# philip-bl/dctn

Measured on AMD Instinct MI355X. Metric: EPS-contraction windows/sec (fwd+bwd), higher is better.
Workload: dtype bf16; 1 GPU; cfg2 EPS[(3,4)]+linear bf16 B1024/GPU; parallelism=dp1

## Files before the change

### dctn_amd/csrc/eps_mfma.hip

```cpp
#include "common.h"

#include <cstdlib>
#include <type_traits>

typedef __attribute__((ext_vector_type(8))) __bf16 bf16x8;
typedef __attribute__((ext_vector_type(16))) float f32x16;
typedef __attribute__((ext_vector_type(8))) float f32x8;
typedef __attribute__((ext_vector_type(2))) int int2v;
typedef __attribute__((ext_vector_type(4))) int int4v;
typedef __attribute__((ext_vector_type(2))) float f32x2;

namespace {

constexpr int ilog2(int v) { return v <= 1 ? 0 : 1 + ilog2(v >> 1); }

template <typename S> __device__ __forceinline__ float to_f32(S v) { return (float)v; }

__device__ __forceinline__ float half_sum(float v) {
  const int iv = __float_as_int(v);
  const int2v r = __builtin_amdgcn_permlane32_swap(iv, iv, false, false);
  return __int_as_float(r[0]) + __int_as_float(r[1]);
}

__device__ __forceinline__ void swap_halves(float& a, float& b) {
// ... 47 lines not shown

struct FastDiv {
  unsigned M, s1, s2;
};
__device__ __forceinline__ unsigned fdiv(unsigned n, const FastDiv& d) {
  const unsigned t = __umulhi(d.M, n);
  return (t + ((n - t) >> d.s1)) >> d.s2;
}

#define MFMA_MAXN 16
struct MfmaP {
  int C, B, K, O, Ho, Wo;
  int P;
  int npg;
  int spc, nchunks;
  unsigned foffb[MFMA_MAXN];
  unsigned rowoffb[MFMA_MAXN];
  unsigned s1b, s2b, s3b, s4b;
  unsigned x_bytes;
  unsigned o_bytes, o_s1b;
  FastDiv div_wo;
  int rowvec_ok;
  int vec_ok;
  int Cout;
  unsigned hw_rowb, hw_bytes;
  int ncb;
  int opts;
#ifdef DCTN_STAMPS
  unsigned long long* stamps;
#endif
};

#ifdef DCTN_STAMPS
#define DCTN_STAMP(P, SLOT)                                                                      \
  do {                                                                                           \
    __builtin_amdgcn_sched_barrier(0);                                                           \
    unsigned long long t_;                                                                       \
    asm volatile("s_memrealtime %0\n\ts_waitcnt lgkmcnt(0)" : "=s"(t_)::"memory");               \
    if ((P).stamps && threadIdx.x == 0) (P).stamps[(long long)blockIdx.x * 8 + (SLOT)] = t_;     \
    __builtin_amdgcn_sched_barrier(0);                                                           \
  } while (0)
static unsigned long long* g_stamps = nullptr;
void dctn_stamps_set(unsigned long long* p) { g_stamps = p; }
__device__ unsigned long long* g_dev_stamps = nullptr;
void dctn_reduce_stamps_set(unsigned long long* p) { (void)hipMemcpyToSymbol(HIP_SYMBOL(g_dev_stamps), &p, sizeof(p)); }
#define DCTN_STAMP_T(P, SLOT, TID)                                                              \
  do {                                                                                           \
    __builtin_amdgcn_sched_barrier(0);                                                           \
    unsigned long long t_;                                                                       \
    asm volatile("s_memrealtime %0\n\ts_waitcnt lgkmcnt(0)" : "=s"(t_)::"memory");               \
    if ((P).stamps && threadIdx.x == (TID)) (P).stamps[(long long)blockIdx.x * 8 + (SLOT)] = t_;  \
    __builtin_amdgcn_sched_barrier(0);                                                           \
  } while (0)
#define DCTN_STAMP_G(SLOT)                                                                       \
  do {                                                                                           \
    __builtin_amdgcn_sched_barrier(0);                                                           \
    unsigned long long t_;                                                                       \
    asm volatile("s_memrealtime %0\n\ts_waitcnt lgkmcnt(0)" : "=s"(t_)::"memory");               \
    if (g_dev_stamps && threadIdx.x == 0) g_dev_stamps[(long long)blockIdx.x * 8 + (SLOT)] = t_;  \
    __builtin_amdgcn_sched_barrier(0);                                                           \
  } while (0)
#else
#define DCTN_STAMP(P, SLOT) do { } while (0)
#define DCTN_STAMP_T(P, SLOT, TID) do { } while (0)
#define DCTN_STAMP_G(SLOT) do { } while (0)
#endif

typedef __attribute__((ext_vector_type(4))) unsigned u32x4;
typedef __attribute__((ext_vector_type(2))) unsigned u32x2;
typedef __attribute__((ext_vector_type(2))) __bf16 bf16x2;

__device__ __forceinline__ __amdgpu_buffer_rsrc_t make_rsrc(const void* ptr, unsigned bytes) {
  return __builtin_amdgcn_make_buffer_rsrc(const_cast<void*>(ptr), 0, (int)bytes, 0x00020000);
}

template <typename S, int N, bool VEC, int ROWS>
struct RawWindow {
  u32x4 row[ROWS > 0 ? ROWS : 1];
  unsigned v[(ROWS == 0 && VEC) ? N * (int)(sizeof(S) / 2) : 1];
  unsigned e[(ROWS == 0 && !VEC) ? 2 * N : 1];
};

template <typename S, int N, bool VEC, int ROWS>
__device__ __forceinline__ void issue_window(__amdgpu_buffer_rsrc_t rs, unsigned voff, unsigned soff,
                                             const MfmaP& p, RawWindow<S, N, VEC, ROWS>& raw) {
  if constexpr (ROWS > 0) {
#pragma unroll
    for (int rw = 0; rw < ROWS; ++rw)
      raw.row[rw] = __builtin_amdgcn_raw_buffer_load_b128(rs, voff, soff + p.rowoffb[rw], 0);
  } else if constexpr (VEC) {
#pragma unroll
    for (int n = 0; n < N; ++n) {
      if constexpr (sizeof(S) == 2) {
        raw.v[n] = __builtin_amdgcn_raw_buffer_load_b32(rs, voff, soff + p.foffb[n], 0);
      } else {
        const u32x2 t = __builtin_amdgcn_raw_buffer_load_b64(rs, voff, soff + p.foffb[n], 0);
        raw.v[2 * n] = t.x;
        raw.v[2 * n + 1] = t.y;
      }
    }
  } else {
#pragma unroll
    for (int n = 0; n < N; ++n)
#pragma unroll
      for (int q = 0; q < 2; ++q) {
        if constexpr (sizeof(S) == 2)
          raw.e[2 * n + q] = (unsigned)(unsigned short)__builtin_amdgcn_raw_buffer_load_b16(
              rs, voff, soff + p.foffb[n] + q * p.s4b, 0);
        else
          raw.e[2 * n + q] = __builtin_amdgcn_raw_buffer_load_b32(rs, voff, soff + p.foffb[n] + q * p.s4b, 0);
      }
  }
}

template <typename S, int N, bool VEC, int ROWS>
__device__ __forceinline__ void unpack_window(const RawWindow<S, N, VEC, ROWS>& raw, float (&xv)[N][2]) {
  if constexpr (ROWS > 0) {
    constexpr int KK = N / ROWS;
// ... 672 lines not shown
    const int nks = (F + 31) / 32;
    const int c = lane & 15, kg = lane >> 4;
    const __amdgpu_buffer_rsrc_t rs_hw = make_rsrc(hw, p.hw_bytes);
    u32x4 wf[HEADT_MAXKS];
#pragma unroll
    for (int i = 0; i < HEADT_MAXKS; ++i) {
      const int ks = wv + HEADT_WAVES * i, k = 32 * ks + 8 * kg;
      const unsigned vo2 = (ks < nks && c < p.Cout && k + 7 < F) ? (unsigned)c * p.hw_rowb + (unsigned)k * 2u : p.hw_bytes;
      wf[i] = __builtin_amdgcn_raw_buffer_load_b128(rs_hw, vo2, 0, 0);
    }
    __syncthreads();
    f32x4v hd = {0.f, 0.f, 0.f, 0.f};
    const short* brd = ftile + (c < HEADT_GS ? c : HEADT_GS - 1) * LP + 8 * kg;
#pragma unroll
    for (int i = 0; i < HEADT_MAXKS; ++i) {
      const int ks = wv + HEADT_WAVES * i;
      if (ks < nks) {
        const bf16x8 fb = *reinterpret_cast<const bf16x8*>(brd + 32 * ks);
        hd = __builtin_amdgcn_mfma_f32_16x16x32_bf16(__builtin_bit_cast(bf16x8, wf[i]), fb, hd, 0, 0, 0);
      }
    }
    if (c < HEADT_GS) {
#pragma unroll
      for (int v = 0; v < 4; ++v) hsum[wv][c][4 * kg + v] = hd[v];
    }
    if constexpr (BLK4) {
      static_assert(HEADT_GS == 4, "a group is one block of the blocked4 layout");
      const unsigned sob = (unsigned)(g0 >> 2) * (unsigned)F * 8u;
      for (int f = 2 * tid; f < F; f += 2 * 64 * HEADT_WAVES) {
        unsigned r[HEADT_GS];
#pragma unroll
        for (int i = 0; i < HEADT_GS; ++i) r[i] = i < ng ? *reinterpret_cast<const unsigned*>(ftile + i * LP + f) : 0u;
        const u32x4 q = u32x4{__builtin_amdgcn_perm(r[1], r[0], 0x05040100u), __builtin_amdgcn_perm(r[3], r[2], 0x05040100u),
                              __builtin_amdgcn_perm(r[1], r[0], 0x07060302u), __builtin_amdgcn_perm(r[3], r[2], 0x07060302u)};
        __builtin_amdgcn_raw_buffer_store_b128(q, rs_o, (unsigned)f * 8u, sob, 0);
      }
    }
    __syncthreads();
    if (tid < HEADT_GS * 16) {
      const int sl = tid >> 4, cc = tid & 15;
      if (sl < ng && cc < p.Cout) {
        float t = (float)bias[cc];
#pragma unroll
        for (int w = 0; w < HEADT_WAVES; ++w) t += hsum[w][sl][cc];
        logits[(long long)(g0 + sl) * p.Cout + cc] = (bf16_t)t;
      }
    }
  }
}

constexpr int BWD_WAVES = 8;
constexpr size_t dcore_dyn_lds_bytes(int mt) { return (size_t)BWD_WAVES * (1 + mt) * 64 * 32 * sizeof(short); }

template <typename S, int N0, int N1, int OP, bool XVEC, bool OVEC, int ROWS, int HEADC>
__global__ __launch_bounds__(64 * BWD_WAVES) void eps_bwd_dcore_q2reg_k(const S* __restrict__ x,
                                                             const S* __restrict__ dY,
                                                             const S* __restrict__ hw,
                                                             const S* __restrict__ feat,
                                                             float* __restrict__ partial,
                                                             float* __restrict__ dwpart, MfmaP p) {
  constexpr int N = N0 + N1, A = 1 << N0, BN = 1 << N1, KS = A / 16, MT = BN * OP / 32;
  constexpr int AT = A >= 32 ? A / 32 : 1;
  constexpr int LOGO = ilog2(OP);
  constexpr bool LDST = A == 32 && MT <= 2;
  __shared__ float red[BWD_WAVES][32 * 32];
  extern __shared__ __attribute__((aligned(16))) unsigned char dsm[];
  const int tid = threadIdx.x, lane = tid & 63, r = lane & 31, h = lane >> 5, wv = tid >> 6;
  DCTN_STAMP(p, 0);
  short* tiles = reinterpret_cast<short*>(dsm) + wv * ((1 + MT) * 64 * LROW);
  const TrLane trl = tr_lane(lane);

  bf16x8 ident[2];
#pragma unroll
  for (int sp = 0; sp < 2; ++sp)
#pragma unroll
    for (int j = 0; j < 8; ++j) ident[sp][j] = (bf16_t)((16 * sp + 8 * h + j == r) ? 1.f : 0.f);

  f32x16 acc[MT][AT];
#pragma unroll
  for (int t = 0; t < MT; ++t)
#pragma unroll
    for (int a = 0; a < AT; ++a)
#pragma unroll
      for (int v = 0; v < 16; ++v) acc[t][a][v] = 0.f;

  const WaveJob job = wave_job(p, BWD_WAVES, (int)sizeof(S), HEADC > 0);
  const __amdgpu_buffer_rsrc_t rs_x = make_rsrc(x, p.x_bytes);
  const __amdgpu_buffer_rsrc_t rs_dy = make_rsrc(HEADC > 0 ? feat : dY, p.o_bytes);
  constexpr bool HEADMM = HEADC > 0 && HEADC <= 16 && LDST && OVEC && XVEC && sizeof(S) == 2 && OP == 4;
  float hwf[HEADC > 0 && !HEADMM ? HEADC : 1][OP];
  float dwacc[HEADC > 0 && !HEADMM ? HEADC : 1][OP];
#pragma unroll
  for (int c = 0; c < (HEADC > 0 && !HEADMM ? HEADC : 1); ++c)
#pragma unroll
    for (int o = 0; o < OP; ++o) dwacc[c][o] = 0.f;
  constexpr int DLW = HEADC > 0 ? HEADC / 2 : 1;
  const unsigned* dl32 = reinterpret_cast<const unsigned*>(dY);
  unsigned dlraw[DLW];
  RawRow<S, OP> rr[HEADC > 0 && !HEADMM ? HEADC : 1];
  constexpr bool LATE = HEADC > 0 && LDST && !HEADMM;
  auto issue_head_weight = [&]() {
    if constexpr (HEADC > 0 && !HEADMM) {
      const __amdgpu_buffer_rsrc_t rs_hw = make_rsrc(hw, p.hw_bytes);
      const unsigned voff_hw = job.valid ? (unsigned)job.pos * (unsigned)(OP * 2) : p.hw_bytes;
#pragma unroll
      for (int c = 0; c < HEADC; ++c)
        issue_row<S, OP, true>(rs_hw, c < p.Cout ? voff_hw : p.hw_bytes, (unsigned)c * p.hw_rowb, OP, rr[c]);
    }
  };
  auto ldst_step = [&](const float (&xv)[N][2], auto&& make_dy) {
    if constexpr (LDST) {
      bf16x8 X[KS], Y[KS];
      build_p0<N0>(xv, X, Y);
      float p1[BN];
      p1[0] = xv[N - 1][0];
      p1[1] = xv[N - 1][1];
#pragma unroll
      for (int u = 1; u < N1; ++u)
#pragma unroll
        for (int bb = (1 << u) - 1; bb >= 0; --bb) {
          const f32x2 pr = bmul2(p1[bb], f32x2{xv[N - 1 - u][0], xv[N - 1 - u][1]});
// ... 330 lines not shown
#pragma unroll
        for (int o = 0; o < OP; ++o) {
          float v = 0.f;
#pragma unroll
          for (int c = 0; c < HEADC; ++c) v = (c == c0 + cc) ? dwacc[c][o] : v;
          red1[wv * SLOT + (cc * 64 + lane) * OP + o] = v;
        }
      __syncthreads();
      for (int e = tid; e < CPR * 64 * OP; e += 64 * BWD_WAVES) {
        float sum = 0.f;
#pragma unroll
        for (int k = 0; k < BWD_WAVES; ++k) sum += red1[k * SLOT + e];
        const int cc = e / (64 * OP), rem = e - cc * (64 * OP);
        const int c = c0 + cc, f = pg * 64 * OP + rem;
        if (cb < p.ncb && c < p.Cout && f < F) dwpart[((long long)cb * p.Cout + c) * F + f] = sum;
      }
    }
  }
  DCTN_STAMP(p, 5);
}

template <typename S>
__global__ __launch_bounds__(256) void eps_bwd_dcore_reduce_k(const float* __restrict__ partial,
                                                              S* __restrict__ dCore, int nblk, int A,
                                                              int BN, int O, int OP, int ACOLS) {
  __shared__ float red[8][32];
  const int tid = threadIdx.x, c = tid & 31, k8 = tid >> 5;
  const long long stride = (long long)BN * OP * ACOLS;
  const long long e = (long long)blockIdx.x * 32 + c;
  float acc[8];
#pragma unroll
  for (int i = 0; i < 8; ++i) acc[i] = 0.f;
  int k = k8;
  for (; k + 56 < nblk; k += 64) {
#pragma unroll
    for (int i = 0; i < 8; ++i) acc[i] += partial[(k + 8 * i) * stride + e];
  }
  for (; k < nblk; k += 8) acc[0] += partial[k * stride + e];
  red[k8][c] = ((acc[0] + acc[1]) + (acc[2] + acc[3])) + ((acc[4] + acc[5]) + (acc[6] + acc[7]));
  __syncthreads();
  if (k8 == 0) {
    float t = 0.f;
#pragma unroll
    for (int i = 0; i < 8; ++i) t += red[i][c];
    const int m = (int)(e / ACOLS), a = (int)(e % ACOLS);
    const int b = m / OP, o = m % OP;
    if (a < A && o < O) dCore[((long long)a * BN + b) * O + o] = (S)t;
  }
}

constexpr int DWG_WAVES = 16;
constexpr int DWG_FW = 32;
constexpr int DWG_BFW = 16;
template <int FW, bool BLK4>
__device__ __forceinline__ void head_dw_gemm_role(const bf16_t* __restrict__ feat, const bf16_t* __restrict__ dL,
                                                  bf16_t* __restrict__ dW, int B, int Cout, long long F, int blk,
                                                  float* __restrict__ lds) {
  typedef __attribute__((ext_vector_type(4))) float f32x4v;
  constexpr int FL = FW / 16;
  static_assert(!BLK4 || FL == 1 || FL == 2, "blocked4 pieces of 8 or 16 bytes");
  const int tid = threadIdx.x, lane = tid & 63, wv = tid >> 6, n = lane & 15, kg = lane >> 4;
  const long long fb = BLK4 ? (long long)(B + 3) / 4 * 4 * F * 2 : (long long)B * F * 2;
  const unsigned f_bytes = (unsigned)fb, dl_bytes = (unsigned)B * (unsigned)Cout * 2u;
  const __amdgpu_buffer_rsrc_t rs_f = make_rsrc(feat, f_bytes), rs_dl = make_rsrc(dL, dl_bytes);
  const long long fcol = (long long)blk * FW + FL * n;
  const bool fok = fcol + FL - 1 < F;
  const int spw = (((B + DWG_WAVES - 1) / DWG_WAVES) + 31) / 32 * 32;
  const int b0 = wv * spw, b1 = b0 + spw < B ? b0 + spw : B;
  f32x4v acc[FL];
#pragma unroll
  for (int j = 0; j < FL; ++j) acc[j] = f32x4v{0.f, 0.f, 0.f, 0.f};
  constexpr int FD = FL >= 2 ? FL / 2 : 1;
  constexpr int NF = BLK4 ? 2 : 8, ND = BLK4 ? 2 * FL : FD;
  unsigned fr[NF][ND], frn[NF][ND];
  unsigned a16[8], a16n[8];
  auto issue = [&](int kb, unsigned (&f)[NF][ND], unsigned (&a)[8]) {
    if constexpr (BLK4) {
#pragma unroll
      for (int h = 0; h < 2; ++h) {
        const int b = kb + 8 * kg + 4 * h;
        const unsigned vo = (b < b1 && fok) ? (unsigned)(((long long)(b >> 2) * F + fcol) * 8) : f_bytes;
        if constexpr (FL == 1) {
          const u32x2 q = __builtin_amdgcn_raw_buffer_load_b64(rs_f, vo, 0, 0);
          f[h][0] = q.x;
          f[h][ND - 1] = q.y;
        } else {
          const u32x4 q = __builtin_amdgcn_raw_buffer_load_b128(rs_f, vo, 0, 0);
#pragma unroll
          for (int d = 0; d < 4; ++d) f[h][d] = q[d];
        }
      }
    }
#pragma unroll
    for (int j = 0; j < 8; ++j) {
      const int b = kb + 8 * kg + j;
      const bool in = b < b1;
      if constexpr (!BLK4) {
        const unsigned vo = (in && fok) ? (unsigned)((long long)b * F * 2 + fcol * 2) : f_bytes;
        if constexpr (FL == 1) {
          f[j][0] = (unsigned)(unsigned short)__builtin_amdgcn_raw_buffer_load_b16(rs_f, vo, 0, 0);
        } else if constexpr (FL == 2) {
          f[j][0] = __builtin_amdgcn_raw_buffer_load_b32(rs_f, vo, 0, 0);
        } else {
          const u32x2 q = __builtin_amdgcn_raw_buffer_load_b64(rs_f, vo, 0, 0);
          f[j][0] = q.x;
          f[j][FD - 1] = q.y;
        }
      }
      a[j] = (unsigned)(unsigned short)__builtin_amdgcn_raw_buffer_load_b16(
          rs_dl, (in && n < Cout) ? (unsigned)b * (unsigned)Cout * 2u + 2u * n : dl_bytes, 0, 0);
    }
  };
  DCTN_STAMP_G(0);
  if (b0 < b1) issue(b0, fr, a16);
  for (int kb = b0; kb < b1; kb += 32) {
    if (kb + 32 < b1) issue(kb + 32, frn, a16n);
    __builtin_amdgcn_sched_barrier(0);
    int4v at;
#pragma unroll
    for (int d = 0; d < 4; ++d) at[d] = (int)(a16[2 * d] | (a16[2 * d + 1] << 16));
#pragma unroll
    for (int j = 0; j < FL; ++j) {
      int4v bf;
      if constexpr (BLK4) {
#pragma unroll
        for (int d = 0; d < 4; ++d) bf[d] = (int)fr[d >> 1][2 * j + (d & 1)];
      } else {
        const unsigned sel = (j & 1) ? 0x07060302u : 0x05040100u;
#pragma unroll
        for (int d = 0; d < 4; ++d)
          bf[d] = FL == 1 ? (int)(fr[2 * d][0] | (fr[2 * d + 1][0] << 16))
                          : (int)__builtin_amdgcn_perm(fr[2 * d + 1][j >> 1], fr[2 * d][j >> 1], sel);
      }
      acc[j] = __builtin_amdgcn_mfma_f32_16x16x32_bf16(__builtin_bit_cast(bf16x8, at), __builtin_bit_cast(bf16x8, bf), acc[j], 0, 0, 0);
    }
#pragma unroll
    for (int j = 0; j < NF; ++j)
#pragma unroll
      for (int e = 0; e < ND; ++e) fr[j][e] = frn[j][e];
#pragma unroll
    for (int j = 0; j < 8; ++j) a16[j] = a16n[j];
  }
#pragma unroll
  for (int j = 0; j < FL; ++j)
#pragma unroll
    for (int i = 0; i < 4; ++i) lds[(wv * (4 * FL) + j * 4 + i) * 64 + lane] = acc[j][i];
  DCTN_STAMP_G(1);
  __syncthreads();
  DCTN_STAMP_G(2);
  if (tid < 4 * FL * 64) {
    const int slot = tid >> 6, j = slot >> 2, i = slot & 3;
    float t = 0.f;
#pragma unroll
    for (int w = 0; w < DWG_WAVES; ++w) t += lds[(w * (4 * FL) + slot) * 64 + lane];
    const int c = 4 * kg + i;
    const long long f = (long long)blk * FW + FL * n + j;
    if (c < Cout && f < F) dW[(long long)c * F + f] = (bf16_t)t;
  }
  DCTN_STAMP_G(4);
}

__global__ __launch_bounds__(1024) void eps_head_reduce_k(const float* __restrict__ partial,
                                                          bf16_t* __restrict__ dCore, int nblk, int A, int BN,
                                                          int O, int OP, int ACOLS, int n_core,
                                                          const float* __restrict__ dwpart,
                                                          bf16_t* __restrict__ dW, int ncb, long long nW, int n_dw,
                                                          const bf16_t* __restrict__ dL,
                                                          bf16_t* __restrict__ dBias, int B, int Cout,
                                                          const bf16_t* __restrict__ feat, int gemm) {
  __shared__ float red[32][33];
  const int tid = threadIdx.x;
  const int bid = gemm == 2 && (int)blockIdx.x < n_core + n_dw
                      ? ((int)blockIdx.x < n_dw ? n_core + (int)blockIdx.x : (int)blockIdx.x - n_dw)
                      : (int)blockIdx.x;
  if (bid < n_core) {
    DCTN_STAMP_G(0);
    const int c = tid & 31, k32 = tid >> 5;
    const long long stride = (long long)BN * OP * ACOLS;
    const long long e = (long long)bid * 32 + c;
    float acc = 0.f;
    for (int k0 = 0; k0 < nblk; k0 += 256) {
      float v[8];
#pragma unroll
      for (int i = 0; i < 8; ++i) {
        const int k = k0 + k32 + 32 * i;
        const float ld = partial[(k < nblk ? k : nblk - 1) * stride + e];
        v[i] = k < nblk ? ld : 0.f;
      }
      acc += ((v[0] + v[1]) + (v[2] + v[3])) + ((v[4] + v[5]) + (v[6] + v[7]));
    }
    red[k32][c] = acc;
    __syncthreads();
    if (k32 == 0) {
      float t = 0.f;
#pragma unroll
      for (int i = 0; i < 32; ++i) t += red[i][c];
      const int m = (int)(e / ACOLS), a = (int)(e % ACOLS);
      const int b = m / OP, o = m % OP;
      if (a < A && o < O) dCore[((long long)a * BN + b) * O + o] = (bf16_t)t;
    }
    DCTN_STAMP_G(4);
    return;
  }
  if (bid < n_core + n_dw) {
    if (!dW) return;
    if (gemm) {
      extern __shared__ __attribute__((aligned(16))) float gemm_lds[];
      if (gemm == 2) head_dw_gemm_role<DWG_BFW, true>(feat, dL, dW, B, Cout, nW / Cout, bid - n_core, gemm_lds);
      else head_dw_gemm_role<DWG_FW, false>(feat, dL, dW, B, Cout, nW / Cout, bid - n_core, gemm_lds);
      return;
    }
    const long long e = (long long)(bid - n_core) * 256 + (tid >> 2);
// ... 133 lines not shown
  if (chunks < 1) chunks = 1;
  if (chunks > m.B) chunks = m.B;
  m.spc = (int)((m.B + chunks - 1) / chunks);
  m.nchunks = (m.B + m.spc - 1) / m.spc;
  const long long waves = (long long)m.nchunks * m.npg;
  long long blocks = (waves + wpb - 1) / wpb;
  if (blocks >= 8) blocks = (blocks + 7) / 8 * 8;
  return (int)blocks;
}

template <typename S>
bool row_vec_ok(const MfmaP& m, int OP, const void* ptr) {
  return m.O == OP && ((uintptr_t)ptr % 4) == 0 && (OP * sizeof(S)) % 4 == 0;
}

template <typename S, int N0, int N1, int OP>
int fwd_launch_t(const void* x, const void* core, void* out, double* stats, const MfmaP& m_in, hipStream_t st) {
  MfmaP m = m_in;
  const int blocks = plan_waves(m, 4, (long long)FWD_BLOCKS_PER_CU * dctn_dev().cus * 4);
  const bool ovec = out == nullptr || row_vec_ok<S>(m, OP, out);
  const dim3 g((unsigned)blocks), b(256);
  constexpr int NN = N0 + N1;
  constexpr int RW = NN == 9 ? 3 : 4;
  if (m.rowvec_ok && m.vec_ok && ovec && sizeof(S) == 2)
    hipLaunchKernelGGL((eps_fwd_q2reg_k<S, N0, N1, OP, true, true, RW>), g, b, 0, st, (const S*)x,
                       (const S*)core, (S*)out, stats, m);
  else if (m.vec_ok && ovec)
    hipLaunchKernelGGL((eps_fwd_q2reg_k<S, N0, N1, OP, true, true, 0>), g, b, 0, st, (const S*)x,
                       (const S*)core, (S*)out, stats, m);
  else if (m.vec_ok)
    hipLaunchKernelGGL((eps_fwd_q2reg_k<S, N0, N1, OP, true, false, 0>), g, b, 0, st, (const S*)x,
                       (const S*)core, (S*)out, stats, m);
  else
    hipLaunchKernelGGL((eps_fwd_q2reg_k<S, N0, N1, OP, false, false, 0>), g, b, 0, st, (const S*)x,
                       (const S*)core, (S*)out, stats, m);
  DCTN_CHECK_LAUNCH();
  dctn_set_last_kernel("eps_fwd_mfma_q2reg");
  return DCTN_OK;
}

template <typename S, int N0, int N1, int OP>
int bwd_launch_t(const void* x, const void* dY, void* dCore, void* ws, const MfmaP& m_in,
                 hipStream_t st) {
  constexpr int A = 1 << N0, BN = 1 << N1, AT = A >= 32 ? A / 32 : 1;
  constexpr size_t DYN = dcore_dyn_lds<N0, N1, OP>();
  MfmaP m = m_in;
  const int grid = plan_waves(m, BWD_WAVES, (long long)dctn_dev().cus * BWD_WAVES);
  const bool ovec = row_vec_ok<S>(m, OP, dY);
  const dim3 g(grid), b(64 * BWD_WAVES);
  constexpr int NN = N0 + N1;
  constexpr int RW = NN == 9 ? 3 : 4;
  if (m.rowvec_ok && m.vec_ok && ovec && sizeof(S) == 2)
    DCTN_DCORE_LAUNCH((eps_bwd_dcore_q2reg_k<S, N0, N1, OP, true, true, RW, 0>), g, b, DYN, st,
                       (const S*)x, (const S*)dY, (const S*)nullptr, (const S*)nullptr, (float*)ws, (float*)nullptr, m);
  else if (m.vec_ok && ovec)
    DCTN_DCORE_LAUNCH((eps_bwd_dcore_q2reg_k<S, N0, N1, OP, true, true, 0, 0>), g, b, DYN, st,
                       (const S*)x, (const S*)dY, (const S*)nullptr, (const S*)nullptr, (float*)ws, (float*)nullptr, m);
  else if (m.vec_ok)
    DCTN_DCORE_LAUNCH((eps_bwd_dcore_q2reg_k<S, N0, N1, OP, true, false, 0, 0>), g, b, DYN, st,
                       (const S*)x, (const S*)dY, (const S*)nullptr, (const S*)nullptr, (float*)ws, (float*)nullptr, m);
  else
    DCTN_DCORE_LAUNCH((eps_bwd_dcore_q2reg_k<S, N0, N1, OP, false, false, 0, 0>), g, b, DYN, st,
                       (const S*)x, (const S*)dY, (const S*)nullptr, (const S*)nullptr, (float*)ws, (float*)nullptr, m);
  DCTN_CHECK_LAUNCH();
  if (m.opts & DCTN_OPT_MAIN_KERNEL_ONLY) return DCTN_PARTIAL;
  hipLaunchKernelGGL((eps_bwd_dcore_reduce_k<S>), dim3(BN * OP * AT), dim3(256), 0, st,
                     (const float*)ws, (S*)dCore, grid, A, BN, m.O, OP, AT * 32);
  DCTN_CHECK_LAUNCH();
  dctn_set_last_kernel("eps_bwd_mfma_q2reg");
  return DCTN_OK;
}

int plan_grouped(MfmaP& m) {
  if (m.npg > dctn_dev().cus) return 0;
  long long ncb = dctn_dev().cus / m.npg;
  const long long need = (m.B + BWD_WAVES - 1) / BWD_WAVES;
  if (ncb > need) ncb = need;
  m.spc = (int)((m.B + ncb * BWD_WAVES - 1) / (ncb * BWD_WAVES));
  m.nchunks = (m.B + m.spc - 1) / m.spc;
  m.ncb = (m.nchunks + BWD_WAVES - 1) / BWD_WAVES;
  long long blocks = (long long)m.ncb * m.npg;
  if (blocks >= 8) blocks = (blocks + 7) / 8 * 8;
  return blocks <= dctn_dev().cus ? (int)blocks : 0;
}

size_t head_dw_partial_bytes(const EpsP& p, int Cout) {
  const long long P = (long long)p.Ho * p.Wo, npg = (P + 63) / 64;
  if (npg > dctn_dev().cus) return 0;
  return (size_t)(dctn_dev().cus / npg) * ((size_t)Cout * (size_t)(P * p.O) + 16) * sizeof(float);
}

long long blocked4_bytes(const MfmaP& m) { return (long long)(m.B + 3) / 4 * 4 * m.P * m.O * 2; }
template <int N0, int N1, int OP>
bool head_blocked4_ok(const MfmaP& m) {
  constexpr int A = 1 << N0, MT = (1 << N1) * OP / 32;
  const long long F = (long long)m.P * OP;
  return A == 32 && MT <= 2 && OP == 4 && m.vec_ok && blocked4_bytes(m) < (1LL << 31) && !(m.opts & DCTN_OPT_SMALL_CHUNKS) &&
         F % 8 == 0 && F <= (long long)HEADT_WAVES * HEADT_MAXKS * 32;
}

template <int N0, int N1, int OP>
int bwd_head_launch_t(const void* x, const void* dL, const void* hw, const void* feat, void* dCore, void* dW,
                      void* dBias, void* ws, size_t core_ws_bytes, const MfmaP& m_in, hipStream_t st) {
  typedef bf16_t S;
  constexpr int A = 1 << N0, BN = 1 << N1, AT = A >= 32 ? A / 32 : 1;
  constexpr size_t DYN = dcore_dyn_lds<N0, N1, OP>();
  MfmaP m = m_in;
  const bool blk = (m.opts & DCTN_OPT_HEAD_FEATURES_BLOCKED4) != 0;
  if (m.O != OP || m.Cout < 2 || m.Cout > 16 || m.Cout % 2 != 0) return DCTN_ERR_UNSUPPORTED;
  if (((uintptr_t)dL % 4) != 0 || ((uintptr_t)hw % 4) != 0 || ((uintptr_t)feat % (blk ? 16 : 4)) != 0) return DCTN_ERR_UNSUPPORTED;
  if (blk && !head_blocked4_ok<N0, N1, OP>(m)) return DCTN_ERR_UNSUPPORTED;
  const int grid = plan_grouped(m);
  if (grid == 0) return DCTN_ERR_UNSUPPORTED;
  float* dwpart = reinterpret_cast<float*>(static_cast<unsigned char*>(ws) + core_ws_bytes);
  const long long nW = (long long)m.Cout * m.P * OP;
  constexpr int MT = BN * OP / 32;
  const bool headmm = A == 32 && MT <= 2 && OP == 4 && m.vec_ok;
  if (headmm && (long long)m.B * m.P * OP * 2 >= (1LL << 31)) return DCTN_ERR_UNSUPPORTED;
  const bool gemm = headmm;

  const dim3 g(grid), b(64 * BWD_WAVES);
  constexpr int NN = N0 + N1;
  constexpr int RW = NN == 9 ? 3 : 4;
#define DCTN_HEAD_LAUNCH(XV, ROWSV, HC)                                                                        \
  DCTN_DCORE_LAUNCH((eps_bwd_dcore_q2reg_k<S, N0, N1, OP, XV, true, ROWSV, HC>), g, b, (DYN > 0 ? DYN + 8192 : 0), st, (const S*)x, \
                     (const S*)dL, (const S*)hw, (const S*)feat, (float*)ws, dwpart, m)
  if (m.rowvec_ok && m.vec_ok) {
    if (m.Cout <= 10) DCTN_HEAD_LAUNCH(true, RW, 10); else DCTN_HEAD_LAUNCH(true, RW, 16);
  } else if (m.vec_ok) {
    if (m.Cout <= 10) DCTN_HEAD_LAUNCH(true, 0, 10); else DCTN_HEAD_LAUNCH(true, 0, 16);
  } else {
    if (m.Cout <= 10) DCTN_HEAD_LAUNCH(false, 0, 10); else DCTN_HEAD_LAUNCH(false, 0, 16);
  }
#undef DCTN_HEAD_LAUNCH
  DCTN_CHECK_LAUNCH();
  if (m.opts & DCTN_OPT_MAIN_KERNEL_ONLY) return DCTN_PARTIAL;
  const int fw = blk ? DWG_BFW : DWG_FW;
  const int n_core = BN * OP * AT, n_dw = gemm ? (int)(((long long)m.P * OP + fw - 1) / fw) : (int)((nW + 255) / 256);
  const size_t gemm_lds = (size_t)DWG_WAVES * (fw / 4) * 64 * sizeof(float);
  static_assert(DWG_WAVES * 64 == 1024, "the gemm role is the whole workgroup of eps_head_reduce_k");
  if (gemm && !dctn_lds_optin((const void*)eps_head_reduce_k, gemm_lds)) return DCTN_ERR_LAUNCH;
  hipLaunchKernelGGL(eps_head_reduce_k, dim3(n_core + n_dw + 1), dim3(1024), gemm ? gemm_lds : 0, st, (const float*)ws, (S*)dCore,
                     grid, A, BN, m.O, OP, AT * 32, n_core, (const float*)dwpart, (S*)dW, m.ncb, nW, n_dw,
                     (const S*)dL, (S*)dBias, m.B, m.Cout, (const S*)feat, gemm ? (blk ? 2 : 1) : 0);
  DCTN_CHECK_LAUNCH();
  dctn_set_last_kernel("eps_head_bwd_mfma_q2reg");
  return DCTN_OK;
}

template <int N0, int N1, int OP>
int fwd_head_launch_t(const void* x, const void* core, const void* hw, const void* bias, void* out, void* logits,
                      const MfmaP& m_in, hipStream_t st) {
  typedef bf16_t S;
  MfmaP m = m_in;
  const bool blk = (m.opts & DCTN_OPT_HEAD_FEATURES_BLOCKED4) != 0;
  if (m.O != OP || !(m.rowvec_ok && m.vec_ok) || m.npg > HEAD_FWD_MAXPG) return DCTN_ERR_UNSUPPORTED;
  if (((uintptr_t)hw % 16) != 0 || m.hw_rowb % 16 != 0 || ((uintptr_t)out % (blk ? 16 : OP * 2)) != 0) return DCTN_ERR_UNSUPPORTED;
  int nwg = m.B < dctn_dev().cus ? m.B : dctn_dev().cus;
  m.spc = (m.B + nwg - 1) / nwg;
  if (blk) m.spc = (m.spc + HEADT_GS - 1) / HEADT_GS * HEADT_GS;
  nwg = (m.B + m.spc - 1) / m.spc;
  constexpr int RW = (N0 + N1) == 9 ? 3 : 4;
  const long long F = (long long)m.P * OP;
  const bool tk = !(m.opts & DCTN_OPT_SMALL_CHUNKS) && F % 8 == 0 && F <= (long long)HEADT_WAVES * HEADT_MAXKS * 32;
  if (blk) {
    if (!tk || !head_blocked4_ok<N0, N1, OP>(m)) return DCTN_ERR_UNSUPPORTED;
    m.o_bytes = blocked4_bytes(m);
  }
  if (tk) {
    const size_t dyn = (size_t)HEADT_GS * headt_pitch((int)F) * sizeof(short);
#define DCTN_HEADT_LAUNCH(BLK)                                                                                          \
    if (!dctn_lds_optin((const void*)eps_fwd_head_q2reg_t_k<N0, N1, OP, RW, BLK>, dyn)) return DCTN_ERR_UNSUPPORTED;    \
    hipLaunchKernelGGL((eps_fwd_head_q2reg_t_k<N0, N1, OP, RW, BLK>), dim3((unsigned)nwg), dim3(64 * HEADT_WAVES), dyn, st, \
                       (const S*)x, (const S*)core, (const S*)hw, (const S*)bias, (S*)out, (S*)logits, m)
    if (blk) { DCTN_HEADT_LAUNCH(true); } else { DCTN_HEADT_LAUNCH(false); }
#undef DCTN_HEADT_LAUNCH
    DCTN_CHECK_LAUNCH();
    dctn_set_last_kernel("eps_head_fwd_mfma_q2reg");
    return DCTN_OK;
  }
  const dim3 g((unsigned)nwg), b((unsigned)(64 * m.npg));
  hipLaunchKernelGGL((eps_fwd_head_q2reg_k<N0, N1, OP, RW>), g, b, 0, st, (const S*)x, (const S*)core, (const S*)hw,
                     (const S*)bias, (S*)out, (S*)logits, m);
  DCTN_CHECK_LAUNCH();
  dctn_set_last_kernel("eps_head_fwd_mfma_q2reg");
  return DCTN_OK;
}

#define DISPATCH_OP(FN, S, N0, N1, OPV, ...)                         \
  switch (OPV) {                                                     \
    case 2: return FN<S, N0, N1, 2>(__VA_ARGS__);                    \
// ... 112 lines not shown
```

Before: 26.16 billion windows/s.

## Fuse head dW GEMM into dcore backward kernel as extra wave role

Adds four extra waves per dcore-backward workgroup that compute the head weight gradient (feat^T·dL GEMM) concurrently with the main dcore waves, using deep 8-block load pipelining and cooperative/solo slice scheduling. The dW work is dropped from the subsequent reduce kernel, which then only handles the core gradient and bias. The intent is to overlap the dW GEMM with the main backward kernel instead of serializing it in the reduce launch. In exchange the workgroup grows to 12 waves with more LDS, which can lower occupancy or steal issue slots from the main waves. The dW loader is also refactored into shared helpers with 32-bit dL loads plus perm.

```diff
diff --git a/dctn_amd/csrc/eps_mfma.hip b/dctn_amd/csrc/eps_mfma.hip
--- a/dctn_amd/csrc/eps_mfma.hip
+++ b/dctn_amd/csrc/eps_mfma.hip
@@ -123,6 +123,16 @@
     if ((P).stamps && threadIdx.x == (TID)) (P).stamps[(long long)blockIdx.x * 8 + (SLOT)] = t_;  \
     __builtin_amdgcn_sched_barrier(0);                                                           \
   } while (0)
+#define DCTN_STAMP_ROLE_ROW 1024
+#define DCTN_STAMP_R(P, SLOT)                                                                    \
+  do {                                                                                           \
+    __builtin_amdgcn_sched_barrier(0);                                                           \
+    unsigned long long t_;                                                                       \
+    asm volatile("s_memrealtime %0\n\ts_waitcnt lgkmcnt(0)" : "=s"(t_)::"memory");               \
+    if ((P).stamps && threadIdx.x == 64 * 8)                                                     \
+      (P).stamps[(long long)(DCTN_STAMP_ROLE_ROW + blockIdx.x) * 8 + (SLOT)] = t_;               \
+    __builtin_amdgcn_sched_barrier(0);                                                           \
+  } while (0)
 #define DCTN_STAMP_G(SLOT)                                                                       \
   do {                                                                                           \
     __builtin_amdgcn_sched_barrier(0);                                                           \
@@ -135,6 +145,7 @@
 #define DCTN_STAMP(P, SLOT) do { } while (0)
 #define DCTN_STAMP_T(P, SLOT, TID) do { } while (0)
 #define DCTN_STAMP_G(SLOT) do { } while (0)
+#define DCTN_STAMP_R(P, SLOT) do { } while (0)
 #endif
 
 typedef __attribute__((ext_vector_type(4))) unsigned u32x4;
@@ -913,13 +924,17 @@
 constexpr int BWD_WAVES = 8;
 constexpr size_t dcore_dyn_lds_bytes(int mt) { return (size_t)BWD_WAVES * (1 + mt) * 64 * 32 * sizeof(short); }
 
-template <typename S, int N0, int N1, int OP, bool XVEC, bool OVEC, int ROWS, int HEADC>
-__global__ __launch_bounds__(64 * BWD_WAVES) void eps_bwd_dcore_q2reg_k(const S* __restrict__ x,
+__device__ __forceinline__ void head_dw_role_waves(const bf16_t* __restrict__ feat, const bf16_t* __restrict__ dL,
+                                                   bf16_t* __restrict__ dW, int B, int Cout, long long F, int n_dw,
+                                                   int rw, float* __restrict__ lds, const MfmaP& p);
+template <typename S, int N0, int N1, int OP, bool XVEC, bool OVEC, int ROWS, int HEADC, int DWROLE = 0>
+__global__ __launch_bounds__(64 * (BWD_WAVES + DWROLE)) void eps_bwd_dcore_q2reg_k(const S* __restrict__ x,
                                                              const S* __restrict__ dY,
                                                              const S* __restrict__ hw,
                                                              const S* __restrict__ feat,
                                                              float* __restrict__ partial,
-                                                             float* __restrict__ dwpart, MfmaP p) {
+                                                             float* __restrict__ dwpart, MfmaP p,
+                                                             S* __restrict__ dW, int n_dw) {
   constexpr int N = N0 + N1, A = 1 << N0, BN = 1 << N1, KS = A / 16, MT = BN * OP / 32;
   constexpr int AT = A >= 32 ? A / 32 : 1;
   constexpr int LOGO = ilog2(OP);
@@ -928,6 +943,18 @@
   extern __shared__ __attribute__((aligned(16))) unsigned char dsm[];
   const int tid = threadIdx.x, lane = tid & 63, r = lane & 31, h = lane >> 5, wv = tid >> 6;
   DCTN_STAMP(p, 0);
+  if constexpr (DWROLE > 0) {
+    static_assert(HEADC > 0 && HEADC <= 16 && LDST && OVEC && XVEC && sizeof(S) == 2 && OP == 4, "the dW role rides the HEADMM path");
+    const int rw = __builtin_amdgcn_readfirstlane(wv) - BWD_WAVES;
+    if (rw >= 0) {
+      head_dw_role_waves(feat, dY, dW, p.B, p.Cout, (long long)p.P * OP, n_dw, rw,
+                         reinterpret_cast<float*>(dsm + dcore_dyn_lds_bytes(MT) + 8192), p);
+      return;
+    }
+#ifdef DCTN_DWROLE_PRIO
+    __builtin_amdgcn_s_setprio(DCTN_DWROLE_PRIO);
+#endif
+  }
   short* tiles = reinterpret_cast<short*>(dsm) + wv * ((1 + MT) * 64 * LROW);
   const TrLane trl = tr_lane(lane);
 
@@ -1364,94 +1391,123 @@
 constexpr int DWG_WAVES = 16;
 constexpr int DWG_FW = 32;
 constexpr int DWG_BFW = 16;
+typedef __attribute__((ext_vector_type(4))) float f32x4v;
+template <int FW, bool BLK4>
+struct DwBlock {
+  static constexpr int FL = FW / 16;
+  static constexpr int FD = FL >= 2 ? FL / 2 : 1;
+  static constexpr int NF = BLK4 ? 2 : 8, ND = BLK4 ? 2 * FL : FD;
+  static_assert(!BLK4 || FL == 1 || FL == 2, "blocked4 pieces of 8 or 16 bytes");
+  unsigned f[NF][ND];
+  unsigned a[8];
+};
+template <int NF>
+struct DwLane {
+  unsigned f_bytes, dl_bytes;
+  unsigned frow2, arow;
+  unsigned fo[NF], ao[8];
+  int n, kg;
+  unsigned asel;
+};
+template <int FW, bool BLK4>
+__device__ __forceinline__ DwLane<DwBlock<FW, BLK4>::NF> dw_lane(int B, int Cout, long long F, int blk) {
+  constexpr int FL = FW / 16, NF = DwBlock<FW, BLK4>::NF;
+  const int lane = threadIdx.x & 63;
+  DwLane<NF> l;
+  const long long fb = BLK4 ? (long long)(B + 3) / 4 * 4 * F * 2 : (long long)B * F * 2;
+  l.f_bytes = (unsigned)fb;
+  l.dl_bytes = (unsigned)B * (unsigned)Cout * 2u;
+  l.frow2 = (unsigned)F * 2u;
+  l.arow = (unsigned)Cout * 2u;
+  l.n = lane & 15;
+  l.kg = lane >> 4;
+  l.asel = (l.n & 1) ? 0x07060302u : 0x05040100u;
+  const long long fcol = (long long)blk * FW + FL * l.n;
+  const bool fok = fcol + FL - 1 < F;
+#pragma unroll
+  for (int j = 0; j < NF; ++j)
+    l.fo[j] = !fok ? l.f_bytes : BLK4 ? (unsigned)(((long long)(2 * l.kg + j) * F + fcol) * 8) : (unsigned)((8 * l.kg + j) * F * 2 + fcol * 2);
+#pragma unroll
+  for (int j = 0; j < 8; ++j)
+    l.ao[j] = l.n < Cout ? (unsigned)(8 * l.kg + j) * l.arow + 2u * (unsigned)(l.n & ~1) : l.dl_bytes;
+  return l;
+}
+__device__ __forceinline__ int dw_spw(int B) { return (((B + DWG_WAVES - 1) / DWG_WAVES) + 31) / 32 * 32; }
+template <int FW, bool BLK4>
+__device__ __forceinline__ void dw_block_issue(const __amdgpu_buffer_rsrc_t rs_f, const __amdgpu_buffer_rsrc_t rs_dl,
+                                               const DwLane<DwBlock<FW, BLK4>::NF>& l, int kb, int b1, DwBlock<FW, BLK4>& q) {
+  constexpr int FL = DwBlock<FW, BLK4>::FL, NF = DwBlock<FW, BLK4>::NF, ND = DwBlock<FW, BLK4>::ND;
+  const unsigned so_f = (unsigned)kb * l.frow2, so_a = (unsigned)kb * l.arow;
+  auto loads = [&](auto whole) {
+#pragma unroll
+    for (int j = 0; j < NF; ++j) {
+      const unsigned vo = (decltype(whole)::value || kb + 8 * l.kg + (BLK4 ? 4 : 1) * j < b1) ? l.fo[j] : l.f_bytes;
+      if constexpr (ND == 1 && !BLK4 && FL == 1) {
+        q.f[j][0] = (unsigned)(unsigned short)__builtin_amdgcn_raw_buffer_load_b16(rs_f, vo, so_f, 0);
+      } else if constexpr (ND == 1) {
+        q.f[j][0] = __builtin_amdgcn_raw_buffer_load_b32(rs_f, vo, so_f, 0);
+      } else if constexpr (ND == 2) {
+        const u32x2 v = __builtin_amdgcn_raw_buffer_load_b64(rs_f, vo, so_f, 0);
+        q.f[j][0] = v.x;
+        q.f[j][1] = v.y;
+      } else {
+        const u32x4 v = __builtin_amdgcn_raw_buffer_load_b128(rs_f, vo, so_f, 0);
+#pragma unroll
+        for (int d = 0; d < 4; ++d) q.f[j][d] = v[d];
+      }
+    }
+#pragma unroll
+    for (int j = 0; j < 8; ++j)
+      q.a[j] = __builtin_amdgcn_raw_buffer_load_b32(
+          rs_dl, (decltype(whole)::value || kb + 8 * l.kg + j < b1) ? l.ao[j] : l.dl_bytes, so_a, 0);
+  };
+  if (kb + 32 <= b1) loads(std::true_type{}); else loads(std::false_type{});
+}
+template <int FW, bool BLK4>
+__device__ __forceinline__ void dw_block_mfma(const DwBlock<FW, BLK4>& q, unsigned asel, f32x4v (&acc)[FW / 16]) {
+  constexpr int FL = DwBlock<FW, BLK4>::FL;
+  int4v at;
+#pragma unroll
+  for (int d = 0; d < 4; ++d) at[d] = (int)__builtin_amdgcn_perm(q.a[2 * d + 1], q.a[2 * d], asel);
+#pragma unroll
+  for (int j = 0; j < FL; ++j) {
+    int4v bf;
+    if constexpr (BLK4) {
+#pragma unroll
+      for (int d = 0; d < 4; ++d) bf[d] = (int)q.f[d >> 1][2 * j + (d & 1)];
+    } else {
+      const unsigned sel = (j & 1) ? 0x07060302u : 0x05040100u;
+#pragma unroll
+      for (int d = 0; d < 4; ++d)
+        bf[d] = FL == 1 ? (int)(q.f[2 * d][0] | (q.f[2 * d + 1][0] << 16))
+                        : (int)__builtin_amdgcn_perm(q.f[2 * d + 1][j >> 1], q.f[2 * d][j >> 1], sel);
+    }
+    acc[j] = __builtin_amdgcn_mfma_f32_16x16x32_bf16(__builtin_bit_cast(bf16x8, at), __builtin_bit_cast(bf16x8, bf), acc[j], 0, 0, 0);
+  }
+}
+
 template <int FW, bool BLK4>
 __device__ __forceinline__ void head_dw_gemm_role(const bf16_t* __restrict__ feat, const bf16_t* __restrict__ dL,
                                                   bf16_t* __restrict__ dW, int B, int Cout, long long F, int blk,
                                                   float* __restrict__ lds) {
-  typedef __attribute__((ext_vector_type(4))) float f32x4v;
   constexpr int FL = FW / 16;
-  static_assert(!BLK4 || FL == 1 || FL == 2, "blocked4 pieces of 8 or 16 bytes");
-  const int tid = threadIdx.x, lane = tid & 63, wv = tid >> 6, n = lane & 15, kg = lane >> 4;
-  const long long fb = BLK4 ? (long long)(B + 3) / 4 * 4 * F * 2 : (long long)B * F * 2;
-  const unsigned f_bytes = (unsigned)fb, dl_bytes = (unsigned)B * (unsigned)Cout * 2u;
-  const __amdgpu_buffer_rsrc_t rs_f = make_rsrc(feat, f_bytes), rs_dl = make_rsrc(dL, dl_bytes);
-  const long long fcol = (long long)blk * FW + FL * n;
-  const bool fok = fcol + FL - 1 < F;
-  const int spw = (((B + DWG_WAVES - 1) / DWG_WAVES) + 31) / 32 * 32;
+  const int tid = threadIdx.x, lane = tid & 63, wv = tid >> 6;
+  const auto l = dw_lane<FW, BLK4>(B, Cout, F, blk);
+  const int n = l.n, kg = l.kg;
+  const __amdgpu_buffer_rsrc_t rs_f = make_rsrc(feat, l.f_bytes), rs_dl = make_rsrc(dL, l.dl_bytes);
+  const int spw = dw_spw(B);
   const int b0 = wv * spw, b1 = b0 + spw < B ? b0 + spw : B;
   f32x4v acc[FL];
 #pragma unroll
   for (int j = 0; j < FL; ++j) acc[j] = f32x4v{0.f, 0.f, 0.f, 0.f};
-  constexpr int FD = FL >= 2 ? FL / 2 : 1;
-  constexpr int NF = BLK4 ? 2 : 8, ND = BLK4 ? 2 * FL : FD;
-  unsigned fr[NF][ND], frn[NF][ND];
-  unsigned a16[8], a16n[8];
-  auto issue = [&](int kb, unsigned (&f)[NF][ND], unsigned (&a)[8]) {
-    if constexpr (BLK4) {
-#pragma unroll
-      for (int h = 0; h < 2; ++h) {
-        const int b = kb + 8 * kg + 4 * h;
-        const unsigned vo = (b < b1 && fok) ? (unsigned)(((long long)(b >> 2) * F + fcol) * 8) : f_bytes;
-        if constexpr (FL == 1) {
-          const u32x2 q = __builtin_amdgcn_raw_buffer_load_b64(rs_f, vo, 0, 0);
-          f[h][0] = q.x;
-          f[h][ND - 1] = q.y;
-        } else {
-          const u32x4 q = __builtin_amdgcn_raw_buffer_load_b128(rs_f, vo, 0, 0);
-#pragma unroll
-          for (int d = 0; d < 4; ++d) f[h][d] = q[d];
-        }
-      }
-    }
-#pragma unroll
-    for (int j = 0; j < 8; ++j) {
-      const int b = kb + 8 * kg + j;
-      const bool in = b < b1;
-      if constexpr (!BLK4) {
-        const unsigned vo = (in && fok) ? (unsigned)((long long)b * F * 2 + fcol * 2) : f_bytes;
-        if constexpr (FL == 1) {
-          f[j][0] = (unsigned)(unsigned short)__builtin_amdgcn_raw_buffer_load_b16(rs_f, vo, 0, 0);
-        } else if constexpr (FL == 2) {
-          f[j][0] = __builtin_amdgcn_raw_buffer_load_b32(rs_f, vo, 0, 0);
-        } else {
-          const u32x2 q = __builtin_amdgcn_raw_buffer_load_b64(rs_f, vo, 0, 0);
-          f[j][0] = q.x;
-          f[j][FD - 1] = q.y;
-        }
-      }
-      a[j] = (unsigned)(unsigned short)__builtin_amdgcn_raw_buffer_load_b16(
-          rs_dl, (in && n < Cout) ? (unsigned)b * (unsigned)Cout * 2u + 2u * n : dl_bytes, 0, 0);
-    }
-  };
+  DwBlock<FW, BLK4> cur, nxt;
   DCTN_STAMP_G(0);
-  if (b0 < b1) issue(b0, fr, a16);
+  if (b0 < b1) dw_block_issue<FW, BLK4>(rs_f, rs_dl, l, b0, b1, cur);
   for (int kb = b0; kb < b1; kb += 32) {
-    if (kb + 32 < b1) issue(kb + 32, frn, a16n);
+    if (kb + 32 < b1) dw_block_issue<FW, BLK4>(rs_f, rs_dl, l, kb + 32, b1, nxt);
     __builtin_amdgcn_sched_barrier(0);
-    int4v at;
-#pragma unroll
-    for (int d = 0; d < 4; ++d) at[d] = (int)(a16[2 * d] | (a16[2 * d + 1] << 16));
-#pragma unroll
-    for (int j = 0; j < FL; ++j) {
-      int4v bf;
-      if constexpr (BLK4) {
-#pragma unroll
-        for (int d = 0; d < 4; ++d) bf[d] = (int)fr[d >> 1][2 * j + (d & 1)];
-      } else {
-        const unsigned sel = (j & 1) ? 0x07060302u : 0x05040100u;
-#pragma unroll
-        for (int d = 0; d < 4; ++d)
-          bf[d] = FL == 1 ? (int)(fr[2 * d][0] | (fr[2 * d + 1][0] << 16))
-                          : (int)__builtin_amdgcn_perm(fr[2 * d + 1][j >> 1], fr[2 * d][j >> 1], sel);
-      }
-      acc[j] = __builtin_amdgcn_mfma_f32_16x16x32_bf16(__builtin_bit_cast(bf16x8, at), __builtin_bit_cast(bf16x8, bf), acc[j], 0, 0, 0);
-    }
-#pragma unroll
-    for (int j = 0; j < NF; ++j)
-#pragma unroll
-      for (int e = 0; e < ND; ++e) fr[j][e] = frn[j][e];
-#pragma unroll
-    for (int j = 0; j < 8; ++j) a16[j] = a16n[j];
+    dw_block_mfma<FW, BLK4>(cur, l.asel, acc);
+    cur = nxt;
   }
 #pragma unroll
   for (int j = 0; j < FL; ++j)
@@ -1470,6 +1526,95 @@
     if (c < Cout && f < F) dW[(long long)c * F + f] = (bf16_t)t;
   }
   DCTN_STAMP_G(4);
+}
+
+constexpr int DWR_WAVES = 4, DWR_VPW = DWG_WAVES / DWR_WAVES, DWR_DEPTH = 8;
+constexpr size_t DWR_LDS_BYTES = (size_t)DWG_WAVES * 4 * 64 * sizeof(float);
+static_assert(DWG_BFW == 16, "one tile per virtual wave");
+#ifndef DCTN_DWROLE_EARLY_LOADS
+#define DCTN_DWROLE_EARLY_LOADS 0
+#endif
+__device__ __forceinline__ void head_dw_role_waves(const bf16_t* __restrict__ feat, const bf16_t* __restrict__ dL,
+                                                   bf16_t* __restrict__ dW, int B, int Cout, long long F, int n_dw,
+                                                   int rw, float* __restrict__ lds, const MfmaP& p) {
+  typedef DwBlock<DWG_BFW, true> Blk;
+  const int lane = threadIdx.x & 63;
+  const int nb = dw_spw(B) / 32;
+  const int slice0 = (int)blockIdx.x;
+  const bool coop = slice0 < n_dw;
+  auto l = dw_lane<DWG_BFW, true>(B, Cout, F, slice0);
+  const __amdgpu_buffer_rsrc_t rs_f = make_rsrc(feat, l.f_bytes), rs_dl = make_rsrc(dL, l.dl_bytes);
+  Blk q[DWR_DEPTH];
+  int s = slice0, gi = rw * DWR_VPW * nb, ge = gi + DWR_VPW * nb, gc = gi, kc = 0, vc = rw * DWR_VPW;
+  bool solo = false;
+  auto issue_round = [&]() {
+    const int b1 = 32 * ge < B ? 32 * ge : B;
+#pragma unroll
+    for (int j = 0; j < DWR_DEPTH; ++j) dw_block_issue<DWG_BFW, true>(rs_f, rs_dl, l, 32 * (gi + j), b1, q[j]);
+    gi += DWR_DEPTH;
+  };
+  f32x4v acc[1] = {f32x4v{0.f, 0.f, 0.f, 0.f}};
+  f32x4v t4 = f32x4v{0.f, 0.f, 0.f, 0.f};
+  auto consume_round = [&]() {
+#pragma unroll
+    for (int j = 0; j < DWR_DEPTH; ++j)
+      if (gc < ge) {
+        if (32 * gc < B) dw_block_mfma<DWG_BFW, true>(q[j], l.asel, acc);
+        ++gc;
+        if (++kc == nb) {
+          if (solo) {
+            t4 += acc[0];
+          } else {
+#pragma unroll
+            for (int i = 0; i < 4; ++i) lds[(vc * 4 + i) * 64 + lane] = acc[0][i];
+          }
+          acc[0] = f32x4v{0.f, 0.f, 0.f, 0.f};
+          kc = 0;
+          ++vc;
+        }
+      }
+  };
+  if (DCTN_DWROLE_EARLY_LOADS && coop) issue_round();
+  __builtin_amdgcn_s_barrier();
+  if (coop) {
+    if (!DCTN_DWROLE_EARLY_LOADS) issue_round();
+    DCTN_STAMP_R(p, 0);
+    for (;;) {
+      __builtin_amdgcn_sched_barrier(0);
+      consume_round();
+      if (gc >= ge) {
+        if (solo) {
+          const long long f = (long long)s * DWG_BFW + l.n;
+#pragma unroll
+          for (int i = 0; i < 4; ++i) {
+            const int c = 4 * l.kg + i;
+            if (c < Cout && f < F) dW[(long long)c * F + f] = (bf16_t)t4[i];
+          }
+        } else {
+          DCTN_STAMP_R(p, 1);
+        }
+        s += (int)gridDim.x * (solo ? DWR_WAVES : 1 + rw);
+        if (s >= n_dw) break;
+        solo = true;
+        l = dw_lane<DWG_BFW, true>(B, Cout, F, s);
+        gi = gc = kc = vc = 0;
+        ge = DWG_WAVES * nb;
+        t4 = f32x4v{0.f, 0.f, 0.f, 0.f};
+      }
+      issue_round();
+    }
+  }
+  __syncthreads();
+  __builtin_amdgcn_s_barrier();
+  if (coop) {
+    float t = 0.f;
+#pragma unroll
+    for (int w = 0; w < DWG_WAVES; ++w) t += lds[(w * 4 + rw) * 64 + lane];
+    const int c = 4 * (lane >> 4) + rw;
+    const long long f = (long long)slice0 * DWG_BFW + (lane & 15);
+    if (c < Cout && f < F) dW[(long long)c * F + f] = (bf16_t)t;
+  }
+  DCTN_STAMP_R(p, 2);
 }
 
 __global__ __launch_bounds__(1024) void eps_head_reduce_k(const float* __restrict__ partial,
@@ -1709,16 +1854,16 @@
   constexpr int RW = NN == 9 ? 3 : 4;
   if (m.rowvec_ok && m.vec_ok && ovec && sizeof(S) == 2)
     DCTN_DCORE_LAUNCH((eps_bwd_dcore_q2reg_k<S, N0, N1, OP, true, true, RW, 0>), g, b, DYN, st,
-                       (const S*)x, (const S*)dY, (const S*)nullptr, (const S*)nullptr, (float*)ws, (float*)nullptr, m);
+                       (const S*)x, (const S*)dY, (const S*)nullptr, (const S*)nullptr, (float*)ws, (float*)nullptr, m, (S*)nullptr, 0);
   else if (m.vec_ok && ovec)
     DCTN_DCORE_LAUNCH((eps_bwd_dcore_q2reg_k<S, N0, N1, OP, true, true, 0, 0>), g, b, DYN, st,
-                       (const S*)x, (const S*)dY, (const S*)nullptr, (const S*)nullptr, (float*)ws, (float*)nullptr, m);
+                       (const S*)x, (const S*)dY, (const S*)nullptr, (const S*)nullptr, (float*)ws, (float*)nullptr, m, (S*)nullptr, 0);
   else if (m.vec_ok)
     DCTN_DCORE_LAUNCH((eps_bwd_dcore_q2reg_k<S, N0, N1, OP, true, false, 0, 0>), g, b, DYN, st,
-                       (const S*)x, (const S*)dY, (const S*)nullptr, (const S*)nullptr, (float*)ws, (float*)nullptr, m);
+                       (const S*)x, (const S*)dY, (const S*)nullptr, (const S*)nullptr, (float*)ws, (float*)nullptr, m, (S*)nullptr, 0);
   else
     DCTN_DCORE_LAUNCH((eps_bwd_dcore_q2reg_k<S, N0, N1, OP, false, false, 0, 0>), g, b, DYN, st,
-                       (const S*)x, (const S*)dY, (const S*)nullptr, (const S*)nullptr, (float*)ws, (float*)nullptr, m);
+                       (const S*)x, (const S*)dY, (const S*)nullptr, (const S*)nullptr, (float*)ws, (float*)nullptr, m, (S*)nullptr, 0);
   DCTN_CHECK_LAUNCH();
   if (m.opts & DCTN_OPT_MAIN_KERNEL_ONLY) return DCTN_PARTIAL;
   hipLaunchKernelGGL((eps_bwd_dcore_reduce_k<S>), dim3(BN * OP * AT), dim3(256), 0, st,
@@ -1779,10 +1924,34 @@
   const dim3 g(grid), b(64 * BWD_WAVES);
   constexpr int NN = N0 + N1;
   constexpr int RW = NN == 9 ? 3 : 4;
+  const int n_slices = (int)(((long long)m.P * OP + DWG_BFW - 1) / DWG_BFW);
+  bool dwrole = false;
+  if constexpr (A == 32 && MT <= 2 && OP == 4) {
+    constexpr size_t RDYN = DYN + 8192 + DWR_LDS_BYTES;
+#define DCTN_HEAD_ROLE_LAUNCH(ROWSV, HC)                                                                          \
+  do {                                                                                                            \
+    const void* kfn = (const void*)eps_bwd_dcore_q2reg_k<S, N0, N1, OP, true, true, ROWSV, HC, DWR_WAVES>;        \
+    if (dctn_lds_optin(kfn, RDYN)) {                                                                              \
+      hipLaunchKernelGGL((eps_bwd_dcore_q2reg_k<S, N0, N1, OP, true, true, ROWSV, HC, DWR_WAVES>), g,             \
+                         dim3(64 * (BWD_WAVES + DWR_WAVES)), RDYN, st, (const S*)x, (const S*)dL, (const S*)hw,   \
+                         (const S*)feat, (float*)ws, dwpart, m, (S*)dW, dW ? n_slices : 0);                       \
+      dwrole = true;                                                                                              \
+    }                                                                                                             \
+  } while (0)
+    if (blk && headmm) {
+      if (m.rowvec_ok) {
+        if (m.Cout <= 10) DCTN_HEAD_ROLE_LAUNCH(RW, 10); else DCTN_HEAD_ROLE_LAUNCH(RW, 16);
+      } else {
+        if (m.Cout <= 10) DCTN_HEAD_ROLE_LAUNCH(0, 10); else DCTN_HEAD_ROLE_LAUNCH(0, 16);
+      }
+    }
+#undef DCTN_HEAD_ROLE_LAUNCH
+  }
 #define DCTN_HEAD_LAUNCH(XV, ROWSV, HC)                                                                        \
   DCTN_DCORE_LAUNCH((eps_bwd_dcore_q2reg_k<S, N0, N1, OP, XV, true, ROWSV, HC>), g, b, (DYN > 0 ? DYN + 8192 : 0), st, (const S*)x, \
-                     (const S*)dL, (const S*)hw, (const S*)feat, (float*)ws, dwpart, m)
-  if (m.rowvec_ok && m.vec_ok) {
+                     (const S*)dL, (const S*)hw, (const S*)feat, (float*)ws, dwpart, m, (S*)nullptr, 0)
+  if (dwrole) {
+  } else if (m.rowvec_ok && m.vec_ok) {
     if (m.Cout <= 10) DCTN_HEAD_LAUNCH(true, RW, 10); else DCTN_HEAD_LAUNCH(true, RW, 16);
   } else if (m.vec_ok) {
     if (m.Cout <= 10) DCTN_HEAD_LAUNCH(true, 0, 10); else DCTN_HEAD_LAUNCH(true, 0, 16);
@@ -1793,7 +1962,16 @@
   DCTN_CHECK_LAUNCH();
   if (m.opts & DCTN_OPT_MAIN_KERNEL_ONLY) return DCTN_PARTIAL;
   const int fw = blk ? DWG_BFW : DWG_FW;
-  const int n_core = BN * OP * AT, n_dw = gemm ? (int)(((long long)m.P * OP + fw - 1) / fw) : (int)((nW + 255) / 256);
+  const int n_core = BN * OP * AT;
+  if (dwrole) {
+    hipLaunchKernelGGL(eps_head_reduce_k, dim3(n_core + 1), dim3(1024), 0, st, (const float*)ws, (S*)dCore, grid, A, BN, m.O, OP,
+                       AT * 32, n_core, (const float*)dwpart, (S*)nullptr, m.ncb, nW, 0, (const S*)dL, (S*)dBias, m.B, m.Cout,
+                       (const S*)feat, 0);
+    DCTN_CHECK_LAUNCH();
+    dctn_set_last_kernel("eps_head_bwd_mfma_q2reg");
+    return DCTN_OK;
+  }
+  const int n_dw = gemm ? (int)(((long long)m.P * OP + fw - 1) / fw) : (int)((nW + 255) / 256);
   const size_t gemm_lds = (size_t)DWG_WAVES * (fw / 4) * 64 * sizeof(float);
   static_assert(DWG_WAVES * 64 == 1024, "the gemm role is the whole workgroup of eps_head_reduce_k");
   if (gemm && !dctn_lds_optin((const void*)eps_head_reduce_k, gemm_lds)) return DCTN_ERR_LAUNCH;
```

Measured after the change: 27.74 billion windows/s (median of 6 runs). 1.06x the previous value.
